# Nyrox/raymond

Hardware: AMD Instinct MI355X
Metric: Msamples/s (whole node) + achieved HBM GB/s, 1920x1080 @ 500spp 5-bounce (higher is better)
Workload: dtype f64

## Files before the change

include/raymond_hip_probe.h:

```cpp
#ifndef RAYMOND_HIP_PROBE_H
#define RAYMOND_HIP_PROBE_H

#include "raymond_hip.h"

#ifdef __cplusplus
extern "C" {
#endif

rmd_status rmd_probe_philox4x32_10(rmd_context *ctx, size_t n, const uint32_t *ctr4, const uint32_t *key2, uint32_t *out4);
rmd_status rmd_probe_block_uniforms(rmd_context *ctx, uint64_t seed, size_t n, const uint32_t *pixel, const uint32_t *sample,
                                    const uint32_t *block, double *out5);
rmd_status rmd_probe_sphere_intersect(rmd_context *ctx, size_t n, const double *sphere4, const double *ray6, int32_t *hit, double *t);
rmd_status rmd_probe_sphere_normal(rmd_context *ctx, size_t n, const double *sphere4, const double *ray6, const double *t, double *n3);
rmd_status rmd_probe_plane_intersect(rmd_context *ctx, size_t n, const double *plane6, const double *ray6, int32_t *hit, double *t);
rmd_status rmd_probe_aabb_intersect(rmd_context *ctx, size_t n, const double *aabb6, const double *ray6, int32_t *hit, double *t);
rmd_status rmd_probe_triangle_intersect(rmd_context *ctx, size_t n, const double *pos9, const double *ray6, int32_t *hit, double *t);
rmd_status rmd_probe_triangle_normal(rmd_context *ctx, size_t n, const double *pos9, const double *nrm9, const double *ray6,
                                     const double *t, double *n3);
rmd_status rmd_probe_onb(rmd_context *ctx, size_t n, const double *n3, double *t3, double *b3);
rmd_status rmd_probe_cosine_hemisphere(rmd_context *ctx, size_t n, const double *r1, const double *r2, double *dir3, double *pdf);
rmd_status rmd_probe_importance_sample_ggx(rmd_context *ctx, size_t n, const double *reflect3, const double *rough, const double *r1,
                                           const double *r2, double *dir3);
rmd_status rmd_probe_ggx_distribution(rmd_context *ctx, size_t n, const double *n3, const double *h3, const double *rough, double *out);
rmd_status rmd_probe_geometry_smith(rmd_context *ctx, size_t n, const double *n3, const double *v3, const double *l3,
// ... 3 lines not shown
                                double *root_out, double *inv_root_out);
rmd_status rmd_probe_primary_ray(rmd_context *ctx, size_t n, const rmd_camera *cam, const uint32_t *xy2, const double *u2, double *ray6);
rmd_status rmd_probe_scene_intersect(rmd_context *ctx, const rmd_scene *scene, size_t n, const double *ray6, int32_t *obj, double *t,
                                     uint32_t *sub);
rmd_status rmd_probe_grid_intersect(rmd_context *ctx, const rmd_scene *scene, uint32_t g, size_t n, const double *ray6, int32_t *hit,
                                    double *t, uint32_t *tri);
rmd_status rmd_probe_grid_intersect_deep(rmd_context *ctx, const rmd_scene *scene, uint32_t g, size_t n, const double *ray6, uint32_t cut_lanes,
                                         uint32_t cut_round, uint32_t rays_per_wave, int32_t *hit, double *t, uint32_t *tri);
rmd_status rmd_probe_trace_samples(rmd_context *ctx, const rmd_scene *scene, const rmd_camera *cam, const rmd_settings *settings,
                                   size_t n, const uint32_t *xy2, const uint32_t *sample, double *rgb_out, int32_t *path_obj,
                                   uint32_t *path_sub);

rmd_status rmd_probe_triangle_sphere(size_t n, const double *pos9, double *out5);
rmd_status rmd_probe_primary_candidates(const rmd_camera *cam, const rmd_settings *settings, const rmd_object *objects, uint32_t n_objects, uint32_t n_grids,
                                        int64_t axis_pairs_tunable, size_t n_tiles, const uint32_t *tiles4, uint64_t *launch3, uint64_t *out2);
rmd_status rmd_probe_launch_plan(uint32_t mode, uint32_t grid, size_t n, const uint32_t *in5, uint64_t *out8);
rmd_status rmd_probe_launch_sizes(uint32_t mode, uint32_t grid, uint64_t *out8);
rmd_status rmd_probe_scene_layout(const rmd_scene *scene, uint32_t *n_objects, uint32_t *n_grids, uint32_t *mask_words_total);
#define RMD_PROBE_SCRATCH_FORMS 7u
#define RMD_PROBE_SCRATCH_PARTS 14u
rmd_status rmd_probe_denoise_scratch(uint32_t form, uint32_t width, uint32_t height, uint32_t n_rects, uint32_t guided, uint32_t n_cands, uint64_t n_table,
                                     uint64_t *out3, uint64_t *total);
rmd_status rmd_probe_pretest_pairs(rmd_context *ctx, size_t n, const double *sphere5, const double *pos9, const double *ray6, int32_t *pass,
                                   int32_t *hit, double *t);

#ifdef __cplusplus
}
#endif
#endif
```

raymond_amd/csrc/api.cpp:

```cpp
#define RMD_WITH_HIP 1
#include <algorithm>
#include <cmath>
#include <limits>
#include <cstdio>
#include <cstdlib>
#include <cstring>
#include <new>

#include "internal.hpp"
#include "launch.hpp"

using rmd::bind;

namespace {
thread_local std::string tl_last_error;

rmd_status context_create(int32_t device, hipStream_t stream, bool own_stream, rmd_context **out) {
	if (!out) return rmd::fail(nullptr, RMD_ERR_INVALID_ARGUMENT, "rmd_context_create: null out pointer");
	*out = nullptr;
	int count = 0;
	hipError_t e = hipGetDeviceCount(&count);
	if (e != hipSuccess || count <= 0)
		return rmd::fail(nullptr, RMD_ERR_NO_DEVICE, std::string("no HIP device: ") + (e != hipSuccess ? hipGetErrorString(e) : "device count is 0"));
	if (device < 0 || device >= count) return rmd::fail(nullptr, RMD_ERR_INVALID_ARGUMENT, "rmd_context_create: device ordinal out of range");
// ... 154 lines not shown
bool primary_cull_allowed(const RenderParams &P) {
	CullCamera c;
	for (int a = 0; a < 3; a++) c.pos[a] = P.cam_pos[a];
	c.width = P.width, c.height = P.height, c.aspect = P.aspect, c.tan_half_fov = P.tan_half_fov;
	return P.use_dof == 0u && cull_camera_ok(c);
}

RenderParams make_params(const rmd_context *ctx, const rmd_scene *scene, const rmd_camera *cam, const rmd_settings *st) {
	const double PI = 3.14159265358979323846;
	RenderParams P;
	std::memset(&P, 0, sizeof(P));
	for (int a = 0; a < 3; a++) P.cam_pos[a] = cam->position[a];
	P.width = (double)cam->backbuffer_width;
	P.height = (double)cam->backbuffer_height;
	P.inv_width = rmd::exact_reciprocal(P.width), P.inv_height = rmd::exact_reciprocal(P.height);
	P.aspect = P.width / P.height;
	P.tan_half_fov = std::tan(cam->fov_vert / 2.0 * PI / 180.0);
	P.focal_length = cam->focal_length;
	P.aperture_radius = cam->aperture_radius;
	P.W = cam->backbuffer_width, P.H = cam->backbuffer_height;
	P.bounce_limit = st->bounce_limit;
	P.sample_begin = st->sample_begin, P.sample_count = st->sample_count;
	P.n_objects = scene ? scene->n_objects : 0;
	P.n_grids = scene ? scene->n_grids : 0;
	P.mask_words_total = scene ? scene->mask_words_total : 0;
	P.key0 = (uint32_t)st->seed, P.key1 = (uint32_t)(st->seed >> 32);
	P.use_dof = ((st->flags & RMD_RENDER_DOF) && cam->aperture_radius > 0.0) ? 1u : 0u;
	P.end_black_paths = (st->flags & RMD_RENDER_TRACE_BLACK_PATHS) ? 0u : ((st->flags & RMD_RENDER_END_BLACK_PATHS) || !scene || (scene->n_grids == 0u && scene->regular)) ? 1u : 0u;
	P.shade_last_depth = (scene && !scene->regular) ? 1u : 0u;
	P.axis_pairs = scene ? scene->axis_pairs : 0u;
	P.visit_mask = scene ? scene->visit_mask : ~0ull, P.grid_mask = scene ? scene->grid_mask : ~0ull;
	P.primary_cull = (scene && scene->primary_cull && rmd::primary_cull_allowed(P)) ? 1u : 0u;
	P.fault = ctx ? ctx->d_fault : nullptr;
	P.walk_batch = rmd::kWalkBatchDefault;
	if (ctx && ctx->tunable[RMD_TUNE_WALK_BATCH] > 0) P.walk_batch = (uint32_t)ctx->tunable[RMD_TUNE_WALK_BATCH];
	{
		uint32_t k = rmd::kWalkCutDefault;
		if (ctx && ctx->tunable[RMD_TUNE_WALK_CUT] > 0) k = (uint32_t)std::min<int64_t>(ctx->tunable[RMD_TUNE_WALK_CUT] - 1, 31);
		P.walk_cut = (scene && scene->n_grid_objects == 1u) ? (k | (2u * k) << 8) : 0u;
		P.walk_steps_bound = scene ? scene->walk_steps_bound : 0u;
	}
#if RMD_DIAG
	if (ctx) P.debug_flags = ctx->debug_flags;
#endif
	return P;
// ... 132 lines not shown

extern "C++" rmd_status rmd::derive_scene_objects(rmd_context *ctx, const rmd_object *objects, uint32_t n_objects, uint32_t n_grids, int64_t axis_pairs_tunable, rmd::SceneObjects &out) {
	std::vector<rmd::DevObject> &hobj = out.objs;
	hobj.assign(n_objects, rmd::DevObject{});
	bool regular = true;
	for (uint32_t i = 0; i < n_objects; i++) {
		const rmd_object &o = objects[i];
		rmd::DevObject &d = hobj[i];
		std::memset(&d, 0, sizeof(d));
		if (o.geometry_kind > RMD_GEOM_GRID) return rmd::fail(ctx, RMD_ERR_INVALID_ARGUMENT, "rmd_scene_create: unknown geometry kind");
		if (o.material.kind > RMD_MAT_EMISSION) return rmd::fail(ctx, RMD_ERR_INVALID_ARGUMENT, "rmd_scene_create: unknown material kind");
		if (o.geometry_kind == RMD_GEOM_GRID && o.grid_index >= n_grids) return rmd::fail(ctx, RMD_ERR_INVALID_ARGUMENT, "rmd_scene_create: grid_index out of range");
		d.geometry_kind = o.geometry_kind, d.grid_index = o.grid_index, d.material_kind = o.material.kind;
		for (int a = 0; a < 3; a++) d.origin[a] = o.origin[a], d.normal[a] = o.normal[a], d.color[a] = o.material.color[a];
		d.radius = o.radius;
		if (o.material.kind != RMD_MAT_EMISSION && std::fabs(o.material.roughness) > rmd::kMaxRoughness)
			return rmd::fail(ctx, RMD_ERR_UNSUPPORTED, "rmd_scene_create: |roughness| > 512 is not supported");
		if (o.material.kind != RMD_MAT_EMISSION && o.material.roughness != 0.0 && std::fabs(o.material.roughness) < rmd::kMinRoughness)
			return rmd::fail(ctx, RMD_ERR_UNSUPPORTED, "rmd_scene_create: 0 < |roughness| < 1e-12 is not supported");
		d.roughness = o.material.roughness;
		d.metalness = o.material.kind == RMD_MAT_METAL ? 1.0 : 0.0;
		{
			auto tame = [](double v) { return std::fabs(v) <= 1e150; };
			bool ok = true;
			if (o.geometry_kind != RMD_GEOM_GRID)
				for (int a = 0; a < 3; a++) ok = ok && tame(o.origin[a]);
			if (o.geometry_kind == RMD_GEOM_PLANE)
				for (int a = 0; a < 3; a++) ok = ok && tame(o.normal[a]);
			if (o.geometry_kind == RMD_GEOM_SPHERE) ok = ok && tame(o.radius) && o.radius != 0.0 && o.radius * o.radius > 0.0;
			for (int a = 0; a < 3; a++) ok = ok && tame(o.material.color[a]);
// ... 53 lines not shown
                                    rmd_scene **out) {
	if (rmd_status s = bind(ctx)) return s;
	if (!out || (n_objects && !objects) || (n_grids && !grids)) return rmd::fail(ctx, RMD_ERR_INVALID_ARGUMENT, "rmd_scene_create: null argument");
	rmd::SceneObjects derived;
	if (rmd_status s = rmd::derive_scene_objects(ctx, objects, n_objects, n_grids, ctx->tunable[RMD_TUNE_AXIS_PAIRS], derived)) return s;
	std::vector<rmd::DevObject> &hobj = derived.objs;
	const bool regular = derived.regular;
	const uint32_t axis_pairs = derived.axis_pairs;
	auto sc = std::make_unique<rmd_scene>();
	sc->ctx = ctx, sc->n_objects = n_objects, sc->n_grids = n_grids, sc->regular = regular;
	sc->axis_pairs = axis_pairs;
	rmd::DevObject walls_block;
	std::memset(&walls_block, 0, sizeof(walls_block));
	std::memcpy(&walls_block, derived.walls, sizeof(derived.walls));
	sc->visit_mask = derived.visit_mask, sc->grid_mask = derived.grid_mask;
	sc->primary_cull = regular && n_grids == 0u && ctx->tunable[RMD_TUNE_AXIS_PAIRS] == 0;
	for (uint32_t i = 0; i < n_objects; i++) sc->n_grid_objects += objects[i].geometry_kind == RMD_GEOM_GRID ? 1u : 0u;
	auto upload = [&](const void *src, size_t bytes, void **dst) -> hipError_t {
		*dst = nullptr;
		rmd::DeviceBuffer b;
		hipError_t e = b.alloc(bytes ? bytes : 16);
		if (e != hipSuccess) return e;
		*dst = b.as<void>();
		sc->owned.push_back(std::move(b));
		if (bytes) e = hipMemcpy(*dst, src, bytes, hipMemcpyHostToDevice);
		return e;
	};
	std::vector<rmd::DevGrid> hgrid(n_grids);
	for (uint32_t gi = 0; gi < n_grids; gi++) {
		const rmd_grid_desc &g = grids[gi];
		rmd::DevGrid &d = hgrid[gi];
// ... 264 lines not shown
				std::fprintf(stderr, "[rmd queued stamps, cycles] %s trips=%llu fetch=%llu make_ray=%llu simple=%llu walk=%llu ray_push=%llu classify=%llu stores=%llu\n", kinds[k], h[k * 8 + 7],
				             h[k * 8 + 0], h[k * 8 + 1], h[k * 8 + 2], h[k * 8 + 3], h[k * 8 + 4], h[k * 8 + 5], h[k * 8 + 6]);
			std::fprintf(stderr, "[rmd queued stamps, cycles] inside the walks: init=%llu stepping=%llu entry_wait=%llu scan=%llu (chunk search+load+test)=%llu hits=%llu tail=%llu\n",
			             h[24], h[25], h[26], h[27], h[29], h[30], h[31]);
		} else if (P.debug_flags & 16u)
			std::fprintf(stderr, "[rmd stamps, cycles] wave_total=%llu next_ray=%llu simple=%llu walk=%llu classify=%llu | walk: init=%llu stepping=%llu entry_wait=%llu scan=%llu (chunk search+load+test)=%llu hits=%llu tail=%llu\n",
			             h[0], h[1], h[2], h[3], h[4], h[8], h[9], h[10], h[11], h[13], h[14], h[15]);
		else
			std::fprintf(stderr, "[rmd debug] walk_calls=%llu walkers=%llu calls_with_walkers=%llu rounds=%llu wave_steps=%llu lane_steps=%llu test_rounds=%llu tests=%llu chunks=%llu | main_iterations=%llu live_lanes=%llu lanes_with_ray=%llu | stepping iterations with <= 4 / 8 / 16 lanes: %llu / %llu / %llu, with <= 8 lanes while tests wait: %llu\n",
			             h[0], h[1], h[2], h[3], h[4], h[5], h[6], h[8], h[9], h[10], h[11], h[12], h[7], h[13], h[14], h[15]);
		if ((P.debug_flags & 16u) == 0u)
			std::fprintf(stderr, "[rmd debug] sphere pre-test: pairs passed=%llu full chunks=%llu | pairs dropped that pass the reference's test (flag 64; must be 0)=%llu\n", h[17], h[18], h[16]);
		if ((P.debug_flags & 16u) == 0u && (P.debug_flags & 512u))
			std::fprintf(stderr, "[rmd debug] primary candidates: lanes checked=%llu sphere turns left out=%llu trips with two axis pairs left out=%llu | cleared spheres that register a hit (must be 0)=%llu closest hits that differ from the full visit's (must be 0)=%llu\n",
			             h[32], h[35], h[36], h[33], h[34]);
		if ((P.debug_flags & 16u) == 0u && ctx->last_launch.queued)
			std::fprintf(stderr, "[rmd debug] path queues: rays pushed=%llu (of them walks put aside=%llu) rays held in their lanes=%llu hits pushed=%llu hits held in their lanes=%llu\n", h[19], h[22], h[23], h[20], h[21]);
	}
	return RMD_OK;
}

rmd_status rmd_render_tiles_async(rmd_context *ctx, const rmd_scene *scene, const rmd_camera *camera, const rmd_settings *settings,
                                  const rmd_tile_rect *tiles, uint32_t n_tiles, double *accum_dev) {
	return rmd::guarded(ctx, "rmd_render_tiles", [&] { return render_tiles_async_impl(ctx, scene, camera, settings, tiles, n_tiles, accum_dev, nullptr); });
}

rmd_status rmd_render_tiles_moments_async(rmd_context *ctx, const rmd_scene *scene, const rmd_camera *camera, const rmd_settings *settings,
                                          const rmd_tile_rect *tiles, uint32_t n_tiles, double *accum_dev, double *accum_sq_dev) {
	if (accum_sq_dev != nullptr && accum_sq_dev == accum_dev)
		return rmd::fail(ctx, RMD_ERR_INVALID_ARGUMENT, "rmd_render_tiles_moments: accum_sq_dev must not alias accum_dev");
// ... 312 lines not shown
```

raymond_amd/csrc/device_core.hpp:

```cpp
#pragma once
#include <hip/hip_runtime.h>
#include <stdint.h>

#include "device_types.hpp"

#define RMD_DEV __device__ __forceinline__
#ifndef RMD_OPT_BITOP3
#if defined(__gfx950__) || !defined(__HIP_DEVICE_COMPILE__)
#define RMD_OPT_BITOP3 1
#else
#define RMD_OPT_BITOP3 0
#endif
#endif
#define RMD_GLOBAL __attribute__((address_space(1)))
template <class T>
__device__ __forceinline__ const RMD_GLOBAL T *as_global(const T *p) {
	return (const RMD_GLOBAL T *)p;
}

namespace rmd {

struct V3 {
	double x, y, z;
};
RMD_DEV V3 mk(double x, double y, double z) { return V3{x, y, z}; }
RMD_DEV V3 ld3(const double *p) { return V3{p[0], p[1], p[2]}; }
RMD_DEV V3 ld3(const RMD_GLOBAL double *p) { return V3{p[0], p[1], p[2]}; }
RMD_DEV V3 operator+(V3 a, V3 b) { return {a.x + b.x, a.y + b.y, a.z + b.z}; }
RMD_DEV V3 operator-(V3 a, V3 b) { return {a.x - b.x, a.y - b.y, a.z - b.z}; }
RMD_DEV V3 operator-(V3 a) { return {-a.x, -a.y, -a.z}; }
RMD_DEV V3 operator*(V3 a, double s) { return {a.x * s, a.y * s, a.z * s}; }
RMD_DEV V3 operator*(double s, V3 a) { return {s * a.x, s * a.y, s * a.z}; }
RMD_DEV V3 operator/(V3 a, double s) { return {a.x / s, a.y / s, a.z / s}; }
RMD_DEV V3 hadamard(V3 a, V3 b) { return {a.x * b.x, a.y * b.y, a.z * b.z}; }
RMD_DEV double dot(V3 a, V3 b) { return (a.x * b.x + a.y * b.y) + a.z * b.z; }
RMD_DEV V3 cross(V3 a, V3 b) { return {a.y * b.z - a.z * b.y, a.z * b.x - a.x * b.z, a.x * b.y - a.y * b.x}; }
#define RMD_UNLIKELY(c) __builtin_expect(!!(c), 0)
RMD_DEV double sqrt64(double x) {
	const uint32_t hi = (uint32_t)(__builtin_bit_cast(unsigned long long, x) >> 32);
	if (RMD_UNLIKELY(__ballot(hi - 0x10000000u >= 0x7FF00000u - 0x10000000u) != 0ull)) return __builtin_sqrt(x);
	const double y = __builtin_amdgcn_rsq(x);
	double g = x * y, h = y * 0.5;
	const double r = __builtin_fma(-h, g, 0.5);
	g = __builtin_fma(g, r, g), h = __builtin_fma(h, r, h);
	g = __builtin_fma(__builtin_fma(-g, g, x), h, g);
	g = __builtin_fma(__builtin_fma(-g, g, x), h, g);
	return g;
}
RMD_DEV double length(V3 a) { return sqrt64(dot(a, a)); }
RMD_DEV double fast_rcp(double b) {
	double y = __builtin_amdgcn_rcp(b);
// ... 432 lines not shown
			vec = F;
			N = (((a2 * g1n) * g2n) * n_dot_sw) * hv4;
			Dn = (((g1d * g2d) * denominator) * (1.0 - prob_d)) * (a2 * ndh + 0.0001 * (Dd * hv4));
		}
		const V3 wgt = vec * (N * fast_rcp(Dn));
		T = hadamard(T, wgt);
		ro = in.frag + normal * (diffuse ? scalar_const(0.00001) : scalar_const(0.0001));
		rd = sw;
	}
}
RMD_DEV void shade(const RenderParams &P, V3 normal, V3 frag, V3 color, double roughness, double metal, V3 cam_pos, Rng &rng, V3 &ro, V3 &rd, V3 &T) {
	NextRayShadeIn in{normal, frag, color, roughness, metal};
	next_ray(P, true, false, in, cam_pos, 0u, 0u, rng, ro, rd, T);
}

RMD_DEV void primary_ray(const RenderParams &P, uint32_t xi, uint32_t yi, double u0, double u1, V3 &ro, V3 &rd) {
	double x = (double)xi + (u0 - 0.5);
	double y = (double)yi + (u1 - 0.5);
	const double sx = P.inv_width == P.inv_width ? div_by(x + 0.5, P.width, P.inv_width) : (x + 0.5) / P.width;
	const double sy = P.inv_height == P.inv_height ? div_by(y + 0.5, P.height, P.inv_height) : (y + 0.5) / P.height;
	double px = (2.0 * sx - 1.0) * P.tan_half_fov * P.aspect;
	double py = (1.0 - 2.0 * sy) * P.tan_half_fov;
	ro = ld3(P.cam_pos);
	rd = normalize(mk(px, py, 1.0));
}
RMD_DEV bool thin_lens_from_pinhole(const RenderParams &P, V3 po, V3 pd, Rng &rng, V3 &ro, V3 &rd);
RMD_DEV bool primary_ray_dof(const RenderParams &P, uint32_t xi, uint32_t yi, Rng &rng, V3 &ro, V3 &rd) {
	double u0, u1;
	rng.next2(P.key0, P.key1, u0, u1);
	V3 po, pd;
	primary_ray(P, xi, yi, u0, u1, po, pd);
	return thin_lens_from_pinhole(P, po, pd, rng, ro, rd);
}
RMD_DEV bool thin_lens_from_pinhole(const RenderParams &P, V3 po, V3 pd, Rng &rng, V3 &ro, V3 &rd) {
	V3 pos = ld3(P.cam_pos);
// ... 19 lines not shown
```

raymond_amd/csrc/device_types.hpp:

```cpp
#pragma once
#include <stdint.h>

namespace rmd {

struct alignas(16) DevObject {
	uint32_t geometry_kind;
	uint32_t grid_index;
	uint32_t material_kind;
	uint32_t pair_info;
	double origin[3];
	double radius;
	double normal[3];
	double roughness;
	double color[3];
	double metalness;
	uint32_t flags;
	uint32_t _pad2;
	double partner_origin_k;
};
constexpr uint32_t kObjBlackDiffuse = 1u;
constexpr uint32_t kObjAxisPair = 2u, kObjAxisShift = 8u, kObjAxisEarlierIsPlus = 1u << 10;
static_assert(sizeof(DevObject) == 128, "DevObject layout");
constexpr uint32_t kPairTestedAtPartner = 0x80000000u;
constexpr uint32_t kPairAxis = 0x40000000u;

struct alignas(32) AxisWalls {
	double o_plus, o_minus;
	uint32_t idx_plus, idx_minus, _pad[2];
};
static_assert(sizeof(AxisWalls) == 32 && 3 * sizeof(AxisWalls) <= sizeof(DevObject), "the block behind the object table");

struct CellEntry {
	uint32_t first, count;
// ... 51 lines not shown
	uint32_t walk_batch;
	uint32_t mask_words_total;
	uint32_t split_k;
	double *sample_buf;
	uint32_t debug_flags;
	unsigned long long *debug_counters;
	uint32_t *work_counter;
	uint32_t *tile_done;
	uint32_t end_black_paths;
	uint32_t walk_cut;
	uint32_t shade_last_depth;
	uint32_t chain_items;
	uint32_t primary_cull;
	uint32_t buffered;
	uint32_t axis_pairs;
	uint32_t _pad2;
	uint32_t *fault;
	unsigned char *queue_buf;
	uint32_t queue_wave_bytes;
	uint32_t queue_paths;
	uint32_t walk_steps_bound;
	uint32_t _pad3;
	unsigned long long visit_mask;
	unsigned long long grid_mask;
	unsigned long long sample_magic;
};
constexpr uint32_t kFaultTripLoop = 1u;
constexpr uint32_t kFaultSortedTripLoop = 2u;
constexpr uint32_t kFaultWorkLoop = 4u;
constexpr uint32_t kFaultWalkRounds = 8u;
constexpr uint32_t kFaultQueuedTripLoop = 16u;
constexpr uint32_t kFaultWords = 4u;
constexpr uint32_t kWorkCounterPoison = 0x80000000u;

struct ListWork {
	uint32_t x, y, sample, _pad;
};
// ... 3 lines not shown
```

raymond_amd/csrc/internal.hpp:

```cpp
#pragma once
#include <stdint.h>

#include <cmath>
#include <limits>
#include <algorithm>
#include <cstring>

#include <memory>
#include <mutex>
#include <string>
#include <vector>

#include "../../include/raymond_hip.h"

#ifdef RMD_WITH_HIP
#include <hip/hip_runtime_api.h>

#include "device_types.hpp"
#include "primary_candidates.hpp"

#define RMD_HIP(ctx, call)                                                                                      \
	do {                                                                                                        \
		hipError_t e_ = (call);                                                                                 \
		if (e_ != hipSuccess) return rmd::fail(ctx, e_ == hipErrorOutOfMemory ? RMD_ERR_OUT_OF_MEMORY : RMD_ERR_HIP, \
// ... 65 lines not shown
	int64_t tunable[RMD_TUNE_COUNT] = {};
	uint32_t debug_flags = 0;
	rmd_launch_info last_launch = {};
	~rmd_context();
};

struct rmd_scene {
	rmd_context *ctx = nullptr;
	uint32_t n_objects = 0, n_grids = 0;
	uint32_t n_grid_objects = 0;
	uint32_t mask_words_total = 0;
	uint32_t axis_pairs = 0;
	unsigned long long visit_mask = ~0ull, grid_mask = ~0ull;
	uint32_t walk_steps_bound = 0;
	bool primary_cull = false;
	bool regular = true;
	rmd::DevObject *d_objects = nullptr;
	rmd::DevGrid *d_grids = nullptr;
	std::vector<rmd::DeviceBuffer> owned;
	~rmd_scene();
};
#endif

struct rmd_grid_build {
	double bbox_min[3], bbox_max[3], cell_size[3];
	uint32_t res[3];
	std::vector<uint32_t> cells, mapping;
	std::vector<double> pos, nrm;
	std::shared_ptr<void> derived;
	std::mutex derived_mutex;
// ... 95 lines not shown
```

raymond_amd/csrc/probe.cpp:

```cpp
#define RMD_WITH_HIP 1
#include <cstring>
#include <vector>

#include "../../include/raymond_hip_probe.h"
#include "internal.hpp"
#include "launch.hpp"

namespace {

struct Column {
	const double *src;
	int width;
};

rmd_status run_probe(rmd_context *ctx, int op, size_t n, const std::vector<Column> &cols, int out_stride, std::vector<double> &out,
                     const rmd::RenderParams *params = nullptr) {
	if (!ctx) return rmd::fail(nullptr, RMD_ERR_INVALID_ARGUMENT, "probe: null context");
	RMD_HIP(ctx, hipSetDevice(ctx->device));
	int in_stride = 0;
	for (const Column &c : cols) {
		if (!c.src && n) return rmd::fail(ctx, RMD_ERR_INVALID_ARGUMENT, "probe: null input array");
		in_stride += c.width;
	}
	std::vector<double> in(n * in_stride);
// ... 231 lines not shown
			uint64_t visit = sc.visit_mask;
			uint32_t pairs = sc.axis_pairs;
			if (on) {
				if (t[2] == 0u || t[2] > 8u || t[3] == 0u || t[3] > 8u || t[0] > 65535u || t[1] > 65535u) return rmd::fail(nullptr, RMD_ERR_INVALID_ARGUMENT, "probe: a wave tile is 1..8 pixels a side");
				const rmd::TileCone cone = rmd::primary_tile_cone(cc, t[0], t[1], t[2], t[3]);
				for (uint32_t j = 0; j < n_objects && j < 64u; j++)
					if (sc.objs[j].geometry_kind == 1u && rmd::primary_sphere_cleared(cone, cc, sc.objs[j].origin, sc.objs[j].radius)) visit &= ~(1ull << j);
				pairs = rmd::primary_pairs_kept(cone, cc, sc.walls, sc.axis_pairs);
			}
			out2[i * 2] = visit, out2[i * 2 + 1] = pairs;
		}
		return RMD_OK;
	});
}

rmd_status rmd_probe_launch_plan(uint32_t mode, uint32_t grid, size_t n, const uint32_t *in5, uint64_t *out8) {
	if (mode > 2u || grid > 1u || (n != 0 && (!in5 || !out8))) return rmd::fail(nullptr, RMD_ERR_INVALID_ARGUMENT, "probe: bad argument");
	for (size_t i = 0; i < n; i++) {
		const uint32_t *a = in5 + i * 5;
		const rmd::LaunchPlan L = rmd::plan_render_launch((int)mode, grid != 0u, a[0], a[1], (a[2] & 1u) != 0u, (a[2] & 2u) != 0u, (a[2] & 4u) != 0u,
		                                                  (a[2] & 8u) != 0u, a[3], a[4]);
		uint64_t *o = out8 + i * 8;
		o[0] = L.persistent, o[1] = L.queued, o[2] = L.chained, o[3] = L.moments, o[4] = L.waves_per_wg, o[5] = L.workgroups, o[6] = L.wave_lds, o[7] = L.lds;
	}
	return RMD_OK;
}

rmd_status rmd_probe_launch_sizes(uint32_t mode, uint32_t grid, uint64_t *out8) {
	if (mode > 2u || grid > 1u || !out8) return rmd::fail(nullptr, RMD_ERR_INVALID_ARGUMENT, "probe: bad argument");
	rmd::render_lds_sizes((int)mode, grid != 0u, out8);
// ... 66 lines not shown
```

raymond_amd/csrc/render_kernel.hpp:

```cpp
#pragma once
#include <hip/hip_runtime.h>

#include "device_core.hpp"
#include "grid_walk.hpp"
#include "launch.hpp"
#include "primary_candidates.hpp"
#include "scene_split.hpp"

namespace rmd {

struct alignas(16) PathId {
	uint32_t px[64];
	uint32_t smp[64];
	uint32_t sector[64];
};
__host__ __device__ inline size_t wave_lds_bytes(uint32_t n_grids) { return kWaveHeadBytes + (n_grids ? sizeof(WalkScratch) + 64u * 3u * sizeof(double) + sizeof(WalkCarry) + sizeof(PathId) : 0); }

RMD_DEV uint32_t work_item_of_block(uint32_t b, uint32_t nb) {
	(void)nb;
	return b;
}

RMD_DEV void report_fault(const RenderParams &P, uint32_t code, uint32_t detail) {
	if ((threadIdx.x & 63u) == 0u) {
		if (P.fault != nullptr) {
			__hip_atomic_fetch_or(P.fault, code, __ATOMIC_RELAXED, __HIP_MEMORY_SCOPE_SYSTEM);
			__hip_atomic_store(P.fault + 1, detail, __ATOMIC_RELAXED, __HIP_MEMORY_SCOPE_SYSTEM);
			__hip_atomic_fetch_add(P.fault + 2, 1u, __ATOMIC_RELAXED, __HIP_MEMORY_SCOPE_SYSTEM);
		}
		if (P.work_counter != nullptr) __hip_atomic_fetch_or(P.work_counter, kWorkCounterPoison, __ATOMIC_RELAXED, __HIP_MEMORY_SCOPE_AGENT);
	}
}
constexpr uint32_t kTripBoundPerPair = RMD_MAX_BOUNCE_LIMIT_DEV + 4u;
constexpr uint32_t kStallBound = 1u << 18;

template <bool GRID>
RMD_DEV int scene_intersect_wave(const DevObject *__restrict__ objs, uint32_t n_objects, const DevGrid *__restrict__ grids,
                                 const uint32_t *lds_masks, WalkScratch &scr, bool want, V3 ro, V3 rd, double &t_best, uint32_t &sub_best,
                                 uint32_t axis_pairs, uint32_t debug_flags = 0, unsigned long long *dbg = nullptr, bool arbitrary_rays = false,
                                 unsigned long long turns = ~0ull) {
	double closest = kFMax;
	int best = -1;
	uint32_t sub = 0;
	axis_pairs_visit(objs, n_objects, axis_pairs, want, ro, rd, closest, best, arbitrary_rays);
	if constexpr (!GRID) {
		for (uint32_t i = next_turn(~0u, turns); i < n_objects; i = next_turn(i, turns)) {
			const DevObject &o = objs[i];
			double t;
			bool ok;
			int idx = (int)i;
			if (o.geometry_kind == 0u) {
				if (o.pair_info != 0u) {
					if (o.pair_info & kPairTestedAtPartner) continue;
					const uint32_t e = o.pair_info - 1u;
					bool first;
					ok = plane_pair_test_flat(ld3(objs[e].origin), ld3(objs[e].normal), ld3(o.origin), ld3(o.normal), ro, rd, t, first);
					idx = first ? (int)e : (int)i;
					ok = ok && want && lex_less(t, idx, closest, best);
// ... 558 lines not shown
			n_hit -= n;
			const uint32_t st = stack.state[e];
			item = stack.item[e];
			const uint32_t lb = stack.lobe_bits[e];
			rng.block = st >> 16, rng.lobe_bits = lb & 0x3FFFFFu;
			depth = lb >> 24;
			const DevObject &o = lobjs[active ? (st & 0xFFFFu) : 0u];
			T = mk(stack.T[0][e], stack.T[1][e], stack.T[2][e]);
			const V3 normal = mk(stack.normal[0][e], stack.normal[1][e], stack.normal[2][e]);
			const V3 frag = mk(stack.frag[0][e], stack.frag[1][e], stack.frag[2][e]);
			const uint32_t x = tile.x0 + (item & 7u), y = tile.y0 + ((item >> 3) & 7u);
			rng.pixel = y * Pt.W + x, rng.sample = Pt.sample_begin + pool_first + (item >> 6);
			{
				shade(Pt, normal, frag, ld3(o.color), o.roughness, o.metalness, cam_pos, rng, ro, rd, T);
				depth++;
				const bool black = Pt.end_black_paths != 0u && T.x == 0.0 && T.y == 0.0 && T.z == 0.0;
				failed = active && (depth > Pt.bounce_limit || black);
			}
		} else {
			item = next_item + lane;
			next_item += 64u;
			active = item < pool_items && (item & 7u) < tile.w && ((item >> 3) & 7u) < tile.h;
			const uint32_t x = tile.x0 + (item & 7u), y = tile.y0 + ((item >> 3) & 7u);
			rng.pixel = y * Pt.W + x, rng.sample = Pt.sample_begin + pool_first + (item >> 6);
			T = mk(1.0, 1.0, 1.0);
			{
				double u0, u1;
				rng.next2(Pt.key0, Pt.key1, u0, u1);
				primary_ray(Pt, x, y, u0, u1, ro, rd);
				if (Pt.use_dof) failed = active && !thin_lens_from_pinhole(Pt, ro, rd, rng, ro, rd);
			}
			pairs = (uint32_t)__builtin_amdgcn_readfirstlane((int)item_sets[0]);
			turns = (unsigned long long)(uint32_t)__builtin_amdgcn_readfirstlane((int)item_sets[1]) | (unsigned long long)(uint32_t)__builtin_amdgcn_readfirstlane((int)item_sets[2]) << 32;
		}
		const bool want = active && !failed;
		double t = 0.0;
		uint32_t sub = 0;
		__builtin_amdgcn_s_setprio(kSortObjPrio);
		const int oi = scene_intersect_wave<false>(objs, Pt.n_objects, grids, nullptr, *no_scratch, want, ro, rd, t, sub, pairs, 0u, nullptr, false, turns);
		__builtin_amdgcn_s_setprio(0);
#if RMD_DIAG
		if ((Pt.debug_flags & 512u) && (Pt.debug_flags & 8u) && Pt.debug_counters && !shade_trip) {
			double t_full = 0.0;
			uint32_t sub_full = 0;
			const int oi_full = scene_intersect_wave<false>(objs, Pt.n_objects, grids, nullptr, *no_scratch, want, ro, rd, t_full, sub_full, Pt.axis_pairs, 0u, nullptr, false, Pt.visit_mask);
			const bool differs = want && (oi_full != oi || __builtin_bit_cast(unsigned long long, t_full) != __builtin_bit_cast(unsigned long long, t));
			unsigned long long wrong = 0ull;
			const unsigned long long dropped = Pt.visit_mask & ~turns;
			for (unsigned long long m = dropped; m != 0ull; m &= m - 1ull) {
				const DevObject &o = objs[__builtin_ctzll(m)];
				double ts;
				wrong += (unsigned long long)__popcll(__ballot(want && sphere_test_flat(ld3(o.origin), o.radius, ro, rd, ts)));
			}
			const unsigned long long dm = __ballot(differs), wm = __ballot(want);
			if (lane == 0u) {
				atomicAdd(&Pt.debug_counters[32], (unsigned long long)__popcll(wm)), atomicAdd(&Pt.debug_counters[33], wrong);
				atomicAdd(&Pt.debug_counters[34], (unsigned long long)__popcll(dm)), atomicAdd(&Pt.debug_counters[35], (unsigned long long)__popcll(dropped));
				atomicAdd(&Pt.debug_counters[36], pairs != Pt.axis_pairs ? 1ull : 0ull);
			}
		}
// ... 590 lines not shown
```

raymond_amd/csrc/scene_split.hpp:

```cpp
#pragma once
#include "device_core.hpp"
#include "grid_walk.hpp"

namespace rmd {

RMD_DEV uint32_t next_turn(uint32_t i, unsigned long long &m) {
	if (m != 0ull) {
		i = (uint32_t)__builtin_ctzll(m);
		m &= m - 1ull;
		return i;
	}
	return i + 1u < 64u ? 64u : i + 1u;
}
RMD_DEV bool lex_less(double t, int obj, double t_best, int obj_best) { return (t < t_best) | ((t == t_best) & (obj < obj_best)); }
template <int K>
RMD_DEV void axis_pair_test(const DevObject *__restrict__ objs, const AxisWalls *__restrict__ walls, uint32_t j, bool want, V3 ro, V3 rd, double &closest, int &best, bool arbitrary_rays) {
	const AxisWalls &w = walls[K];
	const double o_plus = w.o_plus, o_minus = w.o_minus;
	const int idx_plus = (int)w.idx_plus, idx_minus = (int)w.idx_minus;
	const double rk = K == 0 ? rd.x : K == 1 ? rd.y : rd.z, pk = K == 0 ? ro.x : K == 1 ? ro.y : ro.z;
	const bool faces_plus = -rk > 1e-6, faces_minus = rk > 1e-6;
	double num_minus = o_minus - pk, num_plus = -(o_plus - pk);
	asm volatile("" : "+v"(num_minus), "+v"(num_plus));
	const double num = faces_minus ? num_minus : num_plus;
	const uint32_t num_hi = (uint32_t)(__builtin_bit_cast(unsigned long long, num) >> 32) & 0x7FFFFFFFu;
	if (RMD_UNLIKELY(arbitrary_rays || (__builtin_amdgcn_ballot_w64(num_hi - 0x14300000u >= 0x6BB00000u - 0x14300000u) & __builtin_amdgcn_ballot_w64(want)) != 0ull)) {
		double t;
		bool first;
		const DevObject &o = objs[j];
		const uint32_t e = o.pair_info & 0x3FFFFFFFu;
		const bool hit = plane_pair_test_flat(ld3(objs[e].origin), ld3(objs[e].normal), ld3(o.origin), ld3(o.normal), ro, rd, t, first);
		const int idx = first ? (int)e : (int)j;
		const bool ok = hit && want && lex_less(t, idx, closest, best);
		closest = ok ? t : closest, best = ok ? idx : best;
		return;
	}
	const double t = div_lean(num, __builtin_fabs(rk));
	const int idx = faces_plus ? idx_plus : idx_minus;
	const bool ok = (faces_plus || faces_minus) && t >= 0.0 && want && lex_less(t, idx, closest, best);
	closest = ok ? t : closest, best = ok ? idx : best;
}
RMD_DEV void axis_pairs_visit(const DevObject *__restrict__ objs, uint32_t n_objects, uint32_t axis_pairs, bool want, V3 ro, V3 rd, double &closest, int &best,
                              bool arbitrary_rays = false) {
	const AxisWalls *walls = reinterpret_cast<const AxisWalls *>(objs + n_objects);
	if (axis_pairs & 1023u) axis_pair_test<0>(objs, walls, (axis_pairs & 1023u) - 1u, want, ro, rd, closest, best, arbitrary_rays);
	if ((axis_pairs >> 10) & 1023u) axis_pair_test<1>(objs, walls, ((axis_pairs >> 10) & 1023u) - 1u, want, ro, rd, closest, best, arbitrary_rays);
	if ((axis_pairs >> 20) & 1023u) axis_pair_test<2>(objs, walls, ((axis_pairs >> 20) & 1023u) - 1u, want, ro, rd, closest, best, arbitrary_rays);
}
RMD_DEV bool intersect_simple(const DevObject *__restrict__ objs, uint32_t n_objects, const DevGrid *__restrict__ grids, bool want, V3 ro, V3 rd,
                              double &closest, int &best, uint32_t axis_pairs, unsigned long long turns = ~0ull) {
	closest = scalar_const(kFMax), best = -1;
	bool enters = false;
	axis_pairs_visit(objs, n_objects, axis_pairs, want, ro, rd, closest, best);
	for (uint32_t i = next_turn(~0u, turns); i < n_objects; i = next_turn(i, turns)) {
// ... 46 lines not shown
```

raymond_amd/probe.py:

```python
import ctypes as C
import os

import numpy as np

from . import abi
from . import lib as _lib

_vp = C.c_void_p
_sz = C.c_size_t
_P = C.POINTER
_SIGS = {
    "rmd_probe_philox4x32_10": [_vp, _sz, _vp, _vp, _vp],
    "rmd_probe_block_uniforms": [_vp, C.c_uint64, _sz, _vp, _vp, _vp, _vp],
    "rmd_probe_sphere_intersect": [_vp, _sz, _vp, _vp, _vp, _vp],
    "rmd_probe_sphere_normal": [_vp, _sz, _vp, _vp, _vp, _vp],
    "rmd_probe_plane_intersect": [_vp, _sz, _vp, _vp, _vp, _vp],
    "rmd_probe_aabb_intersect": [_vp, _sz, _vp, _vp, _vp, _vp],
    "rmd_probe_triangle_intersect": [_vp, _sz, _vp, _vp, _vp, _vp],
    "rmd_probe_triangle_normal": [_vp, _sz, _vp, _vp, _vp, _vp, _vp],
    "rmd_probe_onb": [_vp, _sz, _vp, _vp, _vp],
    "rmd_probe_cosine_hemisphere": [_vp, _sz, _vp, _vp, _vp, _vp],
    "rmd_probe_importance_sample_ggx": [_vp, _sz, _vp, _vp, _vp, _vp, _vp],
    "rmd_probe_ggx_distribution": [_vp, _sz, _vp, _vp, _vp, _vp],
    "rmd_probe_geometry_smith": [_vp, _sz, _vp, _vp, _vp, _vp, _vp],
    "rmd_probe_fresnel_schlick": [_vp, _sz, _vp, _vp, _vp],
    "rmd_probe_primary_ray": [_vp, _sz, _P(abi.Camera), _vp, _vp, _vp],
    "rmd_probe_elementary": [_vp, _sz, _vp, _vp, _vp, _vp, _vp, _vp],
    "rmd_probe_scene_intersect": [_vp, _vp, _sz, _vp, _vp, _vp, _vp],
    "rmd_probe_grid_intersect": [_vp, _vp, C.c_uint32, _sz, _vp, _vp, _vp, _vp],
    "rmd_probe_grid_intersect_deep": [_vp, _vp, C.c_uint32, _sz, _vp, C.c_uint32, C.c_uint32, C.c_uint32, _vp, _vp, _vp],
    "rmd_probe_trace_samples": [_vp, _vp, _P(abi.Camera), _P(abi.Settings), _sz, _vp, _vp, _vp, _vp, _vp],
    "rmd_probe_triangle_sphere": [_sz, _vp, _vp],
    "rmd_probe_pretest_pairs": [_vp, _sz, _vp, _vp, _vp, _vp, _vp, _vp],
    "rmd_probe_primary_candidates": [_P(abi.Camera), _P(abi.Settings), _P(abi.Object), C.c_uint32, C.c_uint32, C.c_int64, _sz, _vp, _vp, _vp],
    "rmd_probe_launch_plan": [C.c_uint32, C.c_uint32, _sz, _vp, _vp],
    "rmd_probe_launch_sizes": [C.c_uint32, C.c_uint32, _vp],
    "rmd_probe_scene_layout": [_vp, _P(C.c_uint32), _P(C.c_uint32), _P(C.c_uint32)],
    "rmd_probe_denoise_scratch": [C.c_uint32] * 6 + [C.c_uint64, _vp, _P(C.c_uint64)],
}
PATH_STRIDE = 17
_ready = False


PROBE_LIB_PATH = os.path.join(os.path.dirname(_lib.LIB_PATH), "libraymond_hip_probe.so")
_probe_lib = None


def _L():
    global _ready, _probe_lib
# ... 143 lines not shown


def primary_candidates(cam, settings, scene, tiles, axis_pairs_tunable=0):
    L = _L()
    objs, n, _descs, ng, keep = scene.flatten()
    tiles = np.ascontiguousarray(tiles, dtype=np.uint32).reshape(-1, 4)
    launch, out = np.zeros(3, dtype=np.uint64), np.zeros((tiles.shape[0], 2), dtype=np.uint64)
    c, s = cam.pod(), settings.pod()
    st = L.rmd_probe_primary_candidates(C.byref(c), C.byref(s), objs, n, ng, int(axis_pairs_tunable), tiles.shape[0], _p(tiles), _p(launch), _p(out))
    del keep
    if st != abi.RMD_OK:
        raise RuntimeError("rmd_probe_primary_candidates: status %d" % st)
    return int(launch[0]), int(launch[1]), bool(launch[2]), out[:, 0].copy(), out[:, 1].astype(np.uint32)


MODE_TILES, MODE_TILES_BUFFERED, MODE_LIST = 0, 1, 2
PLAN_QUEUES, PLAN_PERSIST, PLAN_CHAIN, PLAN_MOMENTS = 1, 2, 4, 8
PLAN_FIELDS = ("persistent", "queued", "chained", "moments", "waves_per_wg", "workgroups", "wave_lds", "lds")
SIZE_FIELDS = ("budget", "object", "wave", "queued_wave", "persist_waves", "grid_waves", "sort_pool", "mask_budget")


def _host_check(st, name):
    if st != abi.RMD_OK:
        raise RuntimeError("%s: status %d" % (name, st))


def launch_plan(mode, grid, n_objects, mask_words_total, flags, n_waves, n_cus):
    L = _L()
    cols = np.broadcast_arrays(*(np.asarray(a, dtype=np.int64) for a in (n_objects, mask_words_total, flags, n_waves, n_cus)))
    inp = np.ascontiguousarray(np.stack([c.ravel() for c in cols], axis=1).astype(np.uint32))
# ... 32 lines not shown
```

Measured before the change: 25150.

## Defer sphere root in closest-hit visit and precompute squared radius

```diff
diff --git a/include/raymond_hip_probe.h b/include/raymond_hip_probe.h
--- a/include/raymond_hip_probe.h
+++ b/include/raymond_hip_probe.h
@@ -41,6 +41,7 @@
 rmd_status rmd_probe_triangle_sphere(size_t n, const double *pos9, double *out5);
 rmd_status rmd_probe_primary_candidates(const rmd_camera *cam, const rmd_settings *settings, const rmd_object *objects, uint32_t n_objects, uint32_t n_grids,
                                         int64_t axis_pairs_tunable, size_t n_tiles, const uint32_t *tiles4, uint64_t *launch3, uint64_t *out2);
+rmd_status rmd_probe_closest_hit_host(const rmd_camera *cam, const rmd_settings *settings, const rmd_object *objects, uint32_t n_objects, double *radius2, double *launch3);
 rmd_status rmd_probe_launch_plan(uint32_t mode, uint32_t grid, size_t n, const uint32_t *in5, uint64_t *out8);
 rmd_status rmd_probe_launch_sizes(uint32_t mode, uint32_t grid, uint64_t *out8);
 rmd_status rmd_probe_scene_layout(const rmd_scene *scene, uint32_t *n_objects, uint32_t *n_grids, uint32_t *mask_words_total);
diff --git a/raymond_amd/csrc/api.cpp b/raymond_amd/csrc/api.cpp
--- a/raymond_amd/csrc/api.cpp
+++ b/raymond_amd/csrc/api.cpp
@@ -192,6 +192,7 @@
 	P.width = (double)cam->backbuffer_width;
 	P.height = (double)cam->backbuffer_height;
 	P.inv_width = rmd::exact_reciprocal(P.width), P.inv_height = rmd::exact_reciprocal(P.height);
+	P.recip_ok = (P.inv_width == P.inv_width && P.inv_height == P.inv_height) ? 1u : 0u;
 	P.aspect = P.width / P.height;
 	P.tan_half_fov = std::tan(cam->fov_vert / 2.0 * PI / 180.0);
 	P.focal_length = cam->focal_length;
@@ -207,6 +208,7 @@
 	P.end_black_paths = (st->flags & RMD_RENDER_TRACE_BLACK_PATHS) ? 0u : ((st->flags & RMD_RENDER_END_BLACK_PATHS) || !scene || (scene->n_grids == 0u && scene->regular)) ? 1u : 0u;
 	P.shade_last_depth = (scene && !scene->regular) ? 1u : 0u;
 	P.axis_pairs = scene ? scene->axis_pairs : 0u;
+	P.visit_form = (scene && scene->visit_previous_form) ? 1u : 0u;
 	P.visit_mask = scene ? scene->visit_mask : ~0ull, P.grid_mask = scene ? scene->grid_mask : ~0ull;
 	P.primary_cull = (scene && scene->primary_cull && rmd::primary_cull_allowed(P)) ? 1u : 0u;
 	P.fault = ctx ? ctx->d_fault : nullptr;
@@ -369,6 +371,7 @@
 		d.geometry_kind = o.geometry_kind, d.grid_index = o.grid_index, d.material_kind = o.material.kind;
 		for (int a = 0; a < 3; a++) d.origin[a] = o.origin[a], d.normal[a] = o.normal[a], d.color[a] = o.material.color[a];
 		d.radius = o.radius;
+		if (o.geometry_kind == RMD_GEOM_SPHERE) d.radius2 = o.radius * o.radius;
 		if (o.material.kind != RMD_MAT_EMISSION && std::fabs(o.material.roughness) > rmd::kMaxRoughness)
 			return rmd::fail(ctx, RMD_ERR_UNSUPPORTED, "rmd_scene_create: |roughness| > 512 is not supported");
 		if (o.material.kind != RMD_MAT_EMISSION && o.material.roughness != 0.0 && std::fabs(o.material.roughness) < rmd::kMinRoughness)
@@ -452,7 +455,8 @@
 	std::memset(&walls_block, 0, sizeof(walls_block));
 	std::memcpy(&walls_block, derived.walls, sizeof(derived.walls));
 	sc->visit_mask = derived.visit_mask, sc->grid_mask = derived.grid_mask;
-	sc->primary_cull = regular && n_grids == 0u && ctx->tunable[RMD_TUNE_AXIS_PAIRS] == 0;
+	sc->primary_cull = regular && n_grids == 0u && (ctx->tunable[RMD_TUNE_AXIS_PAIRS] == 0 || ctx->tunable[RMD_TUNE_AXIS_PAIRS] == 3);
+	sc->visit_previous_form = ctx->tunable[RMD_TUNE_AXIS_PAIRS] == 3;
 	for (uint32_t i = 0; i < n_objects; i++) sc->n_grid_objects += objects[i].geometry_kind == RMD_GEOM_GRID ? 1u : 0u;
 	auto upload = [&](const void *src, size_t bytes, void **dst) -> hipError_t {
 		*dst = nullptr;
@@ -747,6 +751,8 @@
 		if ((P.debug_flags & 16u) == 0u && (P.debug_flags & 512u))
 			std::fprintf(stderr, "[rmd debug] primary candidates: lanes checked=%llu sphere turns left out=%llu trips with two axis pairs left out=%llu | cleared spheres that register a hit (must be 0)=%llu closest hits that differ from the full visit's (must be 0)=%llu\n",
 			             h[32], h[35], h[36], h[33], h[34]);
+		if ((P.debug_flags & 16u) == 0u && scene->n_grids == 0u)
+			std::fprintf(stderr, "[rmd debug] closest hit: visits with the deferred root=%llu of them redone in the earlier form (a lane with two sphere candidates)=%llu\n", h[37], h[38]);
 		if ((P.debug_flags & 16u) == 0u && ctx->last_launch.queued)
 			std::fprintf(stderr, "[rmd debug] path queues: rays pushed=%llu (of them walks put aside=%llu) rays held in their lanes=%llu hits pushed=%llu hits held in their lanes=%llu\n", h[19], h[22], h[23], h[20], h[21]);
 	}
diff --git a/raymond_amd/csrc/device_core.hpp b/raymond_amd/csrc/device_core.hpp
--- a/raymond_amd/csrc/device_core.hpp
+++ b/raymond_amd/csrc/device_core.hpp
@@ -35,6 +35,11 @@
 RMD_DEV V3 hadamard(V3 a, V3 b) { return {a.x * b.x, a.y * b.y, a.z * b.z}; }
 RMD_DEV double dot(V3 a, V3 b) { return (a.x * b.x + a.y * b.y) + a.z * b.z; }
 RMD_DEV V3 cross(V3 a, V3 b) { return {a.y * b.z - a.z * b.y, a.z * b.x - a.x * b.z, a.x * b.y - a.y * b.x}; }
+RMD_DEV bool is_zero3(V3 a) {
+	const unsigned long long x = __builtin_bit_cast(unsigned long long, a.x), y = __builtin_bit_cast(unsigned long long, a.y), z = __builtin_bit_cast(unsigned long long, a.z);
+	const uint32_t lo = (uint32_t)x | (uint32_t)y | (uint32_t)z, hi = (uint32_t)(x >> 32) | (uint32_t)(y >> 32) | (uint32_t)(z >> 32);
+	return ((hi & 0x7FFFFFFFu) | lo) == 0u;
+}
 #define RMD_UNLIKELY(c) __builtin_expect(!!(c), 0)
 RMD_DEV double sqrt64(double x) {
 	const uint32_t hi = (uint32_t)(__builtin_bit_cast(unsigned long long, x) >> 32);
@@ -497,11 +502,17 @@
 	next_ray(P, true, false, in, cam_pos, 0u, 0u, rng, ro, rd, T);
 }
 
-RMD_DEV void primary_ray(const RenderParams &P, uint32_t xi, uint32_t yi, double u0, double u1, V3 &ro, V3 &rd) {
+RMD_DEV void primary_ray(const RenderParams &P, uint32_t xi, uint32_t yi, double u0, double u1, V3 &ro, V3 &rd, bool one_flag = false) {
 	double x = (double)xi + (u0 - 0.5);
 	double y = (double)yi + (u1 - 0.5);
-	const double sx = P.inv_width == P.inv_width ? div_by(x + 0.5, P.width, P.inv_width) : (x + 0.5) / P.width;
-	const double sy = P.inv_height == P.inv_height ? div_by(y + 0.5, P.height, P.inv_height) : (y + 0.5) / P.height;
+	double sx, sy;
+	if (one_flag) {
+		if (P.recip_ok != 0u) sx = div_by(x + 0.5, P.width, P.inv_width), sy = div_by(y + 0.5, P.height, P.inv_height);
+		else sx = (x + 0.5) / P.width, sy = (y + 0.5) / P.height;
+	} else {
+		sx = P.inv_width == P.inv_width ? div_by(x + 0.5, P.width, P.inv_width) : (x + 0.5) / P.width;
+		sy = P.inv_height == P.inv_height ? div_by(y + 0.5, P.height, P.inv_height) : (y + 0.5) / P.height;
+	}
 	double px = (2.0 * sx - 1.0) * P.tan_half_fov * P.aspect;
 	double py = (1.0 - 2.0 * sy) * P.tan_half_fov;
 	ro = ld3(P.cam_pos);
diff --git a/raymond_amd/csrc/device_types.hpp b/raymond_amd/csrc/device_types.hpp
--- a/raymond_amd/csrc/device_types.hpp
+++ b/raymond_amd/csrc/device_types.hpp
@@ -16,7 +16,10 @@
 	double metalness;
 	uint32_t flags;
 	uint32_t _pad2;
-	double partner_origin_k;
+	union {
+		double partner_origin_k;
+		double radius2;
+	};
 };
 constexpr uint32_t kObjBlackDiffuse = 1u;
 constexpr uint32_t kObjAxisPair = 2u, kObjAxisShift = 8u, kObjAxisEarlierIsPlus = 1u << 10;
@@ -98,13 +101,13 @@
 	uint32_t primary_cull;
 	uint32_t buffered;
 	uint32_t axis_pairs;
-	uint32_t _pad2;
+	uint32_t visit_form;
 	uint32_t *fault;
 	unsigned char *queue_buf;
 	uint32_t queue_wave_bytes;
 	uint32_t queue_paths;
 	uint32_t walk_steps_bound;
-	uint32_t _pad3;
+	uint32_t recip_ok;
 	unsigned long long visit_mask;
 	unsigned long long grid_mask;
 	unsigned long long sample_magic;
diff --git a/raymond_amd/csrc/internal.hpp b/raymond_amd/csrc/internal.hpp
--- a/raymond_amd/csrc/internal.hpp
+++ b/raymond_amd/csrc/internal.hpp
@@ -103,6 +103,7 @@
 	unsigned long long visit_mask = ~0ull, grid_mask = ~0ull;
 	uint32_t walk_steps_bound = 0;
 	bool primary_cull = false;
+	bool visit_previous_form = false;
 	bool regular = true;
 	rmd::DevObject *d_objects = nullptr;
 	rmd::DevGrid *d_grids = nullptr;
diff --git a/raymond_amd/csrc/probe.cpp b/raymond_amd/csrc/probe.cpp
--- a/raymond_amd/csrc/probe.cpp
+++ b/raymond_amd/csrc/probe.cpp
@@ -269,6 +269,18 @@
 	});
 }
 
+rmd_status rmd_probe_closest_hit_host(const rmd_camera *cam, const rmd_settings *settings, const rmd_object *objects, uint32_t n_objects, double *radius2, double *launch3) {
+	if (!cam || !settings || (n_objects && (!objects || !radius2)) || !launch3) return rmd::fail(nullptr, RMD_ERR_INVALID_ARGUMENT, "probe: bad argument");
+	return rmd::guarded(nullptr, "rmd_probe_closest_hit_host", [&]() -> rmd_status {
+		rmd::SceneObjects sc;
+		if (rmd_status s = rmd::derive_scene_objects(nullptr, objects, n_objects, 0u, 0, sc)) return s;
+		for (uint32_t i = 0; i < n_objects; i++) radius2[i] = sc.objs[i].geometry_kind == 1u ? sc.objs[i].radius2 : 0.0;
+		const rmd::RenderParams P = rmd::make_params(nullptr, nullptr, cam, settings);
+		launch3[0] = P.inv_width, launch3[1] = P.inv_height, launch3[2] = (double)P.recip_ok;
+		return RMD_OK;
+	});
+}
+
 rmd_status rmd_probe_launch_plan(uint32_t mode, uint32_t grid, size_t n, const uint32_t *in5, uint64_t *out8) {
 	if (mode > 2u || grid > 1u || (n != 0 && (!in5 || !out8))) return rmd::fail(nullptr, RMD_ERR_INVALID_ARGUMENT, "probe: bad argument");
 	for (size_t i = 0; i < n; i++) {
diff --git a/raymond_amd/csrc/render_kernel.hpp b/raymond_amd/csrc/render_kernel.hpp
--- a/raymond_amd/csrc/render_kernel.hpp
+++ b/raymond_amd/csrc/render_kernel.hpp
@@ -1,4 +1,9 @@
 #pragma once
+#ifdef X_NO_DEFER
+#define X_FORM false
+#else
+#define X_FORM (Pt.visit_form == 0u)
+#endif
 #include <hip/hip_runtime.h>
 
 #include "device_core.hpp"
@@ -38,10 +43,75 @@
 RMD_DEV int scene_intersect_wave(const DevObject *__restrict__ objs, uint32_t n_objects, const DevGrid *__restrict__ grids,
                                  const uint32_t *lds_masks, WalkScratch &scr, bool want, V3 ro, V3 rd, double &t_best, uint32_t &sub_best,
                                  uint32_t axis_pairs, uint32_t debug_flags = 0, unsigned long long *dbg = nullptr, bool arbitrary_rays = false,
-                                 unsigned long long turns = ~0ull) {
+                                 unsigned long long turns = ~0ull, bool deferred_root = false) {
 	double closest = kFMax;
 	int best = -1;
 	uint32_t sub = 0;
+	if constexpr (!GRID) {
+		if (deferred_root && !arbitrary_rays) {
+			double pend_t = 0.0, pend_arg = 1.0;
+			int pend_idx = -1;
+			unsigned long long seen = 0ull, twice = 0ull;
+#ifdef X_NO_ITEM3
+			axis_pairs_visit(objs, n_objects, axis_pairs, want, ro, rd, closest, best, false);
+#endif
+			unsigned long long left = turns;
+			for (uint32_t i = next_turn(~0u, left); i < n_objects; i = next_turn(i, left)) {
+				const DevObject &o = objs[i];
+				if (o.geometry_kind == 0u) {
+					double t;
+					bool ok;
+					int idx = (int)i;
+					if (o.pair_info != 0u) {
+						if (o.pair_info & kPairTestedAtPartner) continue;
+						const uint32_t e = o.pair_info - 1u;
+						bool first;
+						ok = plane_pair_test_flat(ld3(objs[e].origin), ld3(objs[e].normal), ld3(o.origin), ld3(o.normal), ro, rd, t, first);
+						idx = first ? (int)e : (int)i;
+						ok = ok && want && lex_less(t, idx, closest, best);
+					} else {
+#ifdef X_NO_ITEM3
+						ok = plane_test_flat(ld3(o.origin), ld3(o.normal), ro, rd, t) && want && lex_less(t, idx, closest, best);
+#else
+						ok = plane_test_flat(ld3(o.origin), ld3(o.normal), ro, rd, t) && want && t < closest;
+#endif
+					}
+					closest = ok ? t : closest, best = ok ? idx : best;
+				} else {
+					const V3 c = ld3(o.origin) - ro;
+					const double t = dot(c, rd);
+					const V3 q = c - t * rd;
+					const double p = dot(q, q);
+#ifdef X_NO_R2
+					const double r2 = o.radius * o.radius;
+#else
+					const double r2 = o.radius2;
+#endif
+					const bool cand = !(p > r2) && want;
+					const unsigned long long cm = __ballot(cand);
+					twice |= cm & seen, seen |= cm;
+					pend_t = cand ? t : pend_t, pend_arg = cand ? r2 - p : pend_arg, pend_idx = cand ? (int)i : pend_idx;
+				}
+			}
+			const bool redo = twice != 0ull;
+#if RMD_DIAG
+			if ((debug_flags & 8u) && dbg && (threadIdx.x & 63u) == 0u) atomicAdd(&dbg[37], 1ull), atomicAdd(&dbg[38], redo ? 1ull : 0ull);
+#endif
+			if (!RMD_UNLIKELY(redo)) {
+				if (seen != 0ull) {
+					const double t = pend_t - sqrt64(pend_arg);
+					const bool ok = pend_idx >= 0 && !(t <= 0.0) && lex_less(t, pend_idx, closest, best);
+					closest = ok ? t : closest, best = ok ? pend_idx : best;
+				}
+#ifndef X_NO_ITEM3
+				axis_pairs_visit(objs, n_objects, axis_pairs, want, ro, rd, closest, best, false);
+#endif
+				t_best = closest, sub_best = 0u;
+				return best;
+			}
+			closest = kFMax, best = -1;
+		}
+	}
 	axis_pairs_visit(objs, n_objects, axis_pairs, want, ro, rd, closest, best, arbitrary_rays);
 	if constexpr (!GRID) {
 		for (uint32_t i = next_turn(~0u, turns); i < n_objects; i = next_turn(i, turns)) {
@@ -630,7 +700,13 @@
 			{
 				shade(Pt, normal, frag, ld3(o.color), o.roughness, o.metalness, cam_pos, rng, ro, rd, T);
 				depth++;
+				
+#ifdef X_OLDBLACK
 				const bool black = Pt.end_black_paths != 0u && T.x == 0.0 && T.y == 0.0 && T.z == 0.0;
+#else
+				const bool black = Pt.end_black_paths != 0u && is_zero3(T);
+#endif
+
 				failed = active && (depth > Pt.bounce_limit || black);
 			}
 		} else {
@@ -643,7 +719,13 @@
 			{
 				double u0, u1;
 				rng.next2(Pt.key0, Pt.key1, u0, u1);
-				primary_ray(Pt, x, y, u0, u1, ro, rd);
+				
+#ifdef X_OLDRECIP
+				primary_ray(Pt, x, y, u0, u1, ro, rd, false);
+#else
+				primary_ray(Pt, x, y, u0, u1, ro, rd, true);
+#endif
+
 				if (Pt.use_dof) failed = active && !thin_lens_from_pinhole(Pt, ro, rd, rng, ro, rd);
 			}
 			pairs = (uint32_t)__builtin_amdgcn_readfirstlane((int)item_sets[0]);
@@ -653,13 +735,18 @@
 		double t = 0.0;
 		uint32_t sub = 0;
 		__builtin_amdgcn_s_setprio(kSortObjPrio);
-		const int oi = scene_intersect_wave<false>(objs, Pt.n_objects, grids, nullptr, *no_scratch, want, ro, rd, t, sub, pairs, 0u, nullptr, false, turns);
+#if RMD_DIAG
+		const int oi = scene_intersect_wave<false>(objs, Pt.n_objects, grids, nullptr, *no_scratch, want, ro, rd, t, sub, pairs, Pt.debug_flags, Pt.debug_counters, false, turns, X_FORM);
+#else
+		const int oi = scene_intersect_wave<false>(objs, Pt.n_objects, grids, nullptr, *no_scratch, want, ro, rd, t, sub, pairs, 0u, nullptr, false, turns, X_FORM);
+#endif
 		__builtin_amdgcn_s_setprio(0);
 #if RMD_DIAG
 		if ((Pt.debug_flags & 512u) && (Pt.debug_flags & 8u) && Pt.debug_counters && !shade_trip) {
 			double t_full = 0.0;
 			uint32_t sub_full = 0;
-			const int oi_full = scene_intersect_wave<false>(objs, Pt.n_objects, grids, nullptr, *no_scratch, want, ro, rd, t_full, sub_full, Pt.axis_pairs, 0u, nullptr, false, Pt.visit_mask);
+			const int oi_full = scene_intersect_wave<false>(objs, Pt.n_objects, grids, nullptr, *no_scratch, want, ro, rd, t_full, sub_full, Pt.axis_pairs, 0u, nullptr, false, Pt.visit_mask,
+			                                                Pt.visit_form == 0u);
 			const bool differs = want && (oi_full != oi || __builtin_bit_cast(unsigned long long, t_full) != __builtin_bit_cast(unsigned long long, t));
 			unsigned long long wrong = 0ull;
 			const unsigned long long dropped = Pt.visit_mask & ~turns;
diff --git a/raymond_amd/csrc/scene_split.hpp b/raymond_amd/csrc/scene_split.hpp
--- a/raymond_amd/csrc/scene_split.hpp
+++ b/raymond_amd/csrc/scene_split.hpp
@@ -19,7 +19,13 @@
 	const double o_plus = w.o_plus, o_minus = w.o_minus;
 	const int idx_plus = (int)w.idx_plus, idx_minus = (int)w.idx_minus;
 	const double rk = K == 0 ? rd.x : K == 1 ? rd.y : rd.z, pk = K == 0 ? ro.x : K == 1 ? ro.y : ro.z;
+#ifdef X_OLDFACING
 	const bool faces_plus = -rk > 1e-6, faces_minus = rk > 1e-6;
+	const bool facing = faces_plus || faces_minus;
+#else
+	const bool facing = __builtin_fabs(rk) > 1e-6, negative = (int32_t)(uint32_t)(__builtin_bit_cast(unsigned long long, rk) >> 32) < 0;
+	const bool faces_plus = facing & negative, faces_minus = facing & !negative;
+#endif
 	double num_minus = o_minus - pk, num_plus = -(o_plus - pk);
 	asm volatile("" : "+v"(num_minus), "+v"(num_plus));
 	const double num = faces_minus ? num_minus : num_plus;
@@ -37,7 +43,7 @@
 	}
 	const double t = div_lean(num, __builtin_fabs(rk));
 	const int idx = faces_plus ? idx_plus : idx_minus;
-	const bool ok = (faces_plus || faces_minus) && t >= 0.0 && want && lex_less(t, idx, closest, best);
+	const bool ok = facing && t >= 0.0 && want && lex_less(t, idx, closest, best);
 	closest = ok ? t : closest, best = ok ? idx : best;
 }
 RMD_DEV void axis_pairs_visit(const DevObject *__restrict__ objs, uint32_t n_objects, uint32_t axis_pairs, bool want, V3 ro, V3 rd, double &closest, int &best,
diff --git a/raymond_amd/probe.py b/raymond_amd/probe.py
--- a/raymond_amd/probe.py
+++ b/raymond_amd/probe.py
@@ -33,6 +33,7 @@
     "rmd_probe_triangle_sphere": [_sz, _vp, _vp],
     "rmd_probe_pretest_pairs": [_vp, _sz, _vp, _vp, _vp, _vp, _vp, _vp],
     "rmd_probe_primary_candidates": [_P(abi.Camera), _P(abi.Settings), _P(abi.Object), C.c_uint32, C.c_uint32, C.c_int64, _sz, _vp, _vp, _vp],
+    "rmd_probe_closest_hit_host": [_P(abi.Camera), _P(abi.Settings), _P(abi.Object), C.c_uint32, _vp, _vp],
     "rmd_probe_launch_plan": [C.c_uint32, C.c_uint32, _sz, _vp, _vp],
     "rmd_probe_launch_sizes": [C.c_uint32, C.c_uint32, _vp],
     "rmd_probe_scene_layout": [_vp, _P(C.c_uint32), _P(C.c_uint32), _P(C.c_uint32)],
@@ -206,6 +207,17 @@
     return int(launch[0]), int(launch[1]), bool(launch[2]), out[:, 0].copy(), out[:, 1].astype(np.uint32)
 
 
+def closest_hit_host(cam, settings, scene):
+    L = _L()
+    objs, n, _descs, _ng, keep = scene.flatten()
+    r2, launch = np.zeros(max(n, 1)), np.zeros(3)
+    c, s = cam.pod(), settings.pod()
+    st = L.rmd_probe_closest_hit_host(C.byref(c), C.byref(s), objs, n, _p(r2), _p(launch))
+    del keep
+    _host_check(st, "rmd_probe_closest_hit_host")
+    return r2[:n].copy(), float(launch[0]), float(launch[1]), bool(launch[2])
+
+
 MODE_TILES, MODE_TILES_BUFFERED, MODE_LIST = 0, 1, 2
 PLAN_QUEUES, PLAN_PERSIST, PLAN_CHAIN, PLAN_MOMENTS = 1, 2, 4, 8
 PLAN_FIELDS = ("persistent", "queued", "chained", "moments", "waves_per_wg", "workgroups", "wave_lds", "lds")
```

New measurement: 24740. -1.6%, worse.
